# fishmarch/MS-SLAM

Hardware: AMD Instinct MI355X
Metric: Mkeypoints/s extract+describe, KITTI-00-like stereo 1241x376, 2000 feat/frame (higher is better)
Workload: dtype u8

## Files before the change

### ms-slam_amd/csrc/extractor.hip

```cpp
#include <hip/hip_runtime.h>

#include <algorithm>
#include <atomic>
#include <chrono>
#include <condition_variable>
#include <cstdio>
#include <cstdlib>
#include <cstring>
#include <cmath>
#include <functional>
#include <memory>
#include <mutex>
#include <string>
#include <thread>
#include <vector>

#include "frame_io.h"
#include "hip_host.h"
#include "host_admission.h"
#include "orb_device.h"
#include "gauss7_stream_device.h"
#include "matcher_device.h"
#include "stereo_rowtable_device.h"

// ... 4 lines not shown
thread_local std::string g_last_error;

const int8_t kPattern[1024] = {
#include "orb_pattern.inc"
};

class Pool {
    struct Job {
        const std::function<void(int)>* fn;
        int n;
        std::atomic<int> next{0}, done{0};
    };

public:
    explicit Pool(int nthreads) {
        for (int i = 0; i < nthreads - 1; i++) workers_.emplace_back([this] { loop(); });
    }
    ~Pool() {
        {
            std::lock_guard<std::mutex> lk(m_);
            stop_ = true;
        }
        cv_.notify_all();
        for (auto& t : workers_) t.join();
    }
    void parallel_for(int n, const std::function<void(int)>& fn) {
        if (n <= 0) return;
        auto job = std::make_shared<Job>();
        job->fn = &fn;
        job->n = n;
        {
            std::lock_guard<std::mutex> lk(m_);
            cur_ = job;
            gen_++;
        }
        cv_.notify_all();
        work(*job);
        std::unique_lock<std::mutex> lk(m_);
        done_cv_.wait(lk, [&] { return job->done.load() >= n; });
        cur_.reset();
    }

private:
    void work(Job& job) {
        for (;;) {
            const int i = job.next.fetch_add(1);
            if (i >= job.n) break;
            (*job.fn)(i);
            if (job.done.fetch_add(1) + 1 == job.n) {
                std::lock_guard<std::mutex> lk(m_);
                done_cv_.notify_all();
            }
        }
    }
    void loop() {
        unsigned seen = 0;
        for (;;) {
            std::shared_ptr<Job> job;
            {
                std::unique_lock<std::mutex> lk(m_);
                cv_.wait(lk, [&] { return stop_ || gen_ != seen; });
                if (stop_) return;
                seen = gen_;
                job = cur_;
            }
            if (job) work(*job);
        }
    }
    std::vector<std::thread> workers_;
    std::mutex m_;
    std::condition_variable cv_, done_cv_;
    std::shared_ptr<Job> cur_;
    unsigned gen_ = 0;
    bool stop_ = false;
};

}

constexpr int kMaxGroups = 4;
struct StreamGroup {
    hipStream_t s = nullptr;
    bool own_stream = false;
    hipEvent_t ev_pyr = nullptr, ev_blur = nullptr;
    hipEvent_t pe[10] = {};
    bool ready = false;
};

struct msorb_extractor {
    int device = 0;
    StreamGroup grp[kMaxGroups];
    int n_groups = 2;
    bool overlap_blur = true;
    OrbParams P;
    Semantics sem;
    hipStream_t stream = nullptr, copy_stream = nullptr;
    struct Knobs { bool serial_pipeline = false, quadtree_host = false, quadtree_global = false, split_no_peer = false, force_peer_pyramid = false, frame_compact = true; int host_threads = 0, frame_fuse = 2; } knobs;
    int lds_per_block = 64 * 1024;
    bool last_prof = false;
    int pending_batch = 0;
    DevBuf<int> d_st_sad, d_st_rows, d_st_list;
    DevBuf<uint8_t> d_st_block, d_st_img;
    DevBuf<uint8_t> d_out1;
    DevBuf<uint8_t> d_gather_pyr;
    DevBuf<int> d_gather_cnt;
    hipEvent_t ev_split = nullptr;
    bool host_pyramid = false;
    hipStream_t pyr_stream = nullptr;
    bool h_pyr_async = false;
    const uint8_t* pair_l0[2] = {nullptr, nullptr};
    int pair_pyramids = 0;
    unsigned long long buffers_epoch = 0;
    hipEvent_t ev_compact = nullptr;
    bool profiling = false;
    float stage_ms[MSORB_N_STAGES] = {};

    FrameGeom G;
    bool geom_valid = false;
    std::vector<int> level_cell_begin;
    LevelScale scales;

    DevBuf<uint8_t> d_pyr, d_blur;
    DevBuf<ResizeTap> d_taps;
    TowerPlan tower;
    std::vector<size_t> tap_x_off, tap_y_off;
    DevBuf<CellDesc> d_cells;
    DevBuf<FastThreadRec> d_ttab;
    DevBuf<int> d_level_cell_begin, d_cell_count, d_cell_off, d_level_count, d_img_total, d_img_base, d_sel_count;
    DevBuf<Cand16> d_slots, d_compact;
    DevBuf<SelRec> d_sel;
    DevBuf<uint16_t> d_label;
    DevBuf<int> d_sel_pt, d_sel_n, d_mono;
    QtLevels qt{};
    bool device_quadtree = true;
    bool qt_global = false;
    DevBuf<char> d_qt_ws;
    DevBuf<uint32_t> d_label_wide;
    bool small_cells = false;
    bool compact_on_host = false;
    bool compact_fixed_stride = false;
    PinBuf<int> h_level_count, h_img_base, h_sel_count, h_mono;
    PinBuf<Cand16> h_compact;
    PinBuf<SelRec> h_sel;
    PinBuf<uint8_t> h_pyr, h_img_pin, h_out_pin, h_gather;
    bool h_pyr_valid = false;
    bool input_direct = true;
    msorb_input_stats in_stats{};

    PyramidView last_pyr{}, last_blur{};
    int last_n_images = 0;
    int last_groups = 1;
    int sel_stride = 0;

    std::unique_ptr<Pool> pool;
};

namespace {

int frame_copy(void* dst, const void* src, size_t bytes, hipMemcpyKind kind, hipStream_t s) {
    HIPCHK(small_copy(dst, src, bytes, kind, s));
    return MSORB_OK;
}
int capacity_of(const msorb_extractor* h) { return h->P.nfeatures + (3 + 16) * h->P.nlevels; }

bool have_hip_device() {
    int n = 0;
    if (hipGetDeviceCount(&n) == hipSuccess && n > 0) return true;
    (void)hipGetLastError();
// ... 236 lines not shown
    if (h->qt_global && (rc = h->d_qt_ws.ensure((size_t)n_images * g.nlevels * quadtree_global_workspace_stride(h->qt)))) return rc;
    if (h->qt_global && (rc = h->d_label_wide.ensure((size_t)n_images * g.slots_per_image))) return rc;
    if ((rc = h->d_mono.ensure(std::max(n_images, 4)))) return rc;
    return MSORB_OK;
}

PyramidView make_view(const msorb_extractor* h, const uint8_t* base, const LevelView* level0) {
    PyramidView v{};
    const FrameGeom& g = h->G;
    v.nlevels = g.nlevels;
    for (int l = 0; l < g.nlevels; l++) {
        v.lv[l].base = base + g.lv[l].plane_off;
        v.lv[l].img_stride = g.pyramid_bytes;
        v.lv[l].pitch = g.lv[l].pitch;
        v.lv[l].w = g.lv[l].w;
        v.lv[l].h = g.lv[l].h;
    }
    if (level0) v.lv[0] = *level0;
    return v;
}

PyramidView make_blur_view(const msorb_extractor* h, const uint8_t* base) {
    PyramidView v{};
    const FrameGeom& g = h->G;
    v.nlevels = g.nlevels;
    for (int l = 0; l < g.nlevels; l++) {
        v.lv[l].base = base + g.lv[l].blur_off;
        v.lv[l].img_stride = g.blur_bytes;
        v.lv[l].pitch = g.lv[l].pitch;
        v.lv[l].w = g.lv[l].w;
        v.lv[l].h = g.lv[l].h;
    }
    return v;
}

int fetch_candidates(msorb_extractor* h, int n_images) {
    const int nl = h->G.nlevels;
    HIPCHK(hipStreamWaitEvent(h->copy_stream, h->ev_compact, 0));
    HIPCHK(hipMemcpyAsync(h->h_level_count.p, h->d_level_count.p, (size_t)n_images * nl * sizeof(int),
                          hipMemcpyDeviceToHost, h->copy_stream));
    HIPCHK(hipMemcpyAsync(h->h_img_base.p, h->d_img_base.p, (size_t)(n_images + 1) * sizeof(int),
                          hipMemcpyDeviceToHost, h->copy_stream));
    HIPCHK(hipStreamSynchronize(h->copy_stream));
    int rc;
    if (h->compact_fixed_stride) {
        std::vector<int> tot(n_images, 0);
        int total = 0;
        for (int i = 0; i < n_images; i++) {
            for (int l = 0; l < nl; l++) tot[i] += h->h_level_count.p[(size_t)i * nl + l];
            total += tot[i];
        }
        if ((rc = h->h_compact.ensure(std::max<size_t>((size_t)total + total / 4, 1024)))) return rc;
        int at = 0;
        for (int i = 0; i < n_images; i++) {
            if (tot[i] > 0)
                HIPCHK(hipMemcpyAsync(h->h_compact.p + at, h->d_compact.p + (size_t)h->h_img_base.p[i], (size_t)tot[i] * sizeof(Cand16),
                                      hipMemcpyDeviceToHost, h->copy_stream));
            h->h_img_base.p[i] = at;
            at += tot[i];
        }
        h->h_img_base.p[n_images] = at;
        HIPCHK(hipStreamSynchronize(h->copy_stream));
        h->compact_on_host = true;
        return MSORB_OK;
    }
    const int total = h->h_img_base.p[n_images];
    if ((rc = h->h_compact.ensure(std::max<size_t>((size_t)total + total / 4, 1024)))) return rc;
    if (total > 0) {
        HIPCHK(hipMemcpyAsync(h->h_compact.p, h->d_compact.p, (size_t)total * sizeof(Cand16), hipMemcpyDeviceToHost,
                              h->copy_stream));
        HIPCHK(hipStreamSynchronize(h->copy_stream));
    }
    h->compact_on_host = true;
    return MSORB_OK;
}

int ensure_group(msorb_extractor* h, int gi) {
    StreamGroup& G = h->grp[gi];
    if (G.ready) return MSORB_OK;
    if (gi == 0) G.s = h->stream;
    else { HIPCHK(hipStreamCreateWithFlags(&G.s, hipStreamNonBlocking)); G.own_stream = true; }
    HIPCHK(hipEventCreateWithFlags(&G.ev_pyr, hipEventDisableTiming));
    HIPCHK(hipEventCreateWithFlags(&G.ev_blur, hipEventDisableTiming));
    for (auto& e : G.pe) HIPCHK(hipEventCreate(&e));
    G.ready = true;
    return MSORB_OK;
}

bool device_pipeline(const msorb_extractor* h) { return h->device_quadtree && !h->knobs.serial_pipeline; }
bool blur_off_main(const msorb_extractor* h) { return h->overlap_blur && !h->knobs.serial_pipeline; }

struct PipelineCall {
    int lap0 = 0, lap1 = 0;
    int capacity = 0;
    msorb_keypoint* d_kps = nullptr;
    uint8_t* d_desc = nullptr;
    int* h_counts = nullptr;
    int* h_mono = nullptr;
    const StereoRowJob* row_job = nullptr;
    bool defer_sync = false;
    bool skip_count_copies = false;
    int pair_pyramids = 0;
};

int host_pyramid_copies(msorb_extractor* h, int n, hipEvent_t after) {
    const FrameGeom& g = h->G;
    int rc;
    if ((rc = h->h_pyr.ensure((size_t)n * g.pyramid_bytes))) return rc;
    if (!h->pyr_stream) HIPCHK(hipStreamCreateWithFlags(&h->pyr_stream, hipStreamNonBlocking));
    if (after) HIPCHK(hipStreamWaitEvent(h->pyr_stream, after, 0));
    if (g.nlevels > 1)
        for (int i = 0; i < n; i++)
            HIPCHK(hipMemcpyAsync(h->h_pyr.p + (size_t)i * g.pyramid_bytes + g.lv[1].plane_off, h->d_pyr.p + (size_t)i * g.pyramid_bytes + g.lv[1].plane_off,
                                  g.pyramid_bytes - g.lv[1].plane_off, hipMemcpyDeviceToHost, h->pyr_stream));
    h->h_pyr_async = true;
    return MSORB_OK;
}

int finish_groups(msorb_extractor* h, int n_images, int* h_counts, int* h_mono, float host_select_ms = -1.f) {
    const int ng = h->last_groups;
    for (int gi = 0; gi < ng; gi++) HIPCHK(hipStreamSynchronize(h->grp[gi].s));
    HIPCHK(hipGetLastError());
    for (int i = 0; i < n_images; i++) {
        if (h->h_sel_count.p[i] < 0) { set_last_error("keypoint capacity exceeded"); return MSORB_E_CAPACITY; }
        h_counts[i] = h->h_sel_count.p[i];
        if (h_mono) h_mono[i] = h->h_mono.p[i];
    }
    if (h->last_prof) {
        const int fast_from = blur_off_main(h) ? 1 : 8;
        const int map[6][3] = {{MSORB_STAGE_PYRAMID, 0, 1}, {MSORB_STAGE_FAST, fast_from, 2}, {MSORB_STAGE_COMPACT, 2, 3},
                               {MSORB_STAGE_BLUR, 7, 8}, {MSORB_STAGE_SELECT, 3, 5}, {MSORB_STAGE_DESCRIBE, 5, 6}};
        for (auto& m : map) h->stage_ms[m[0]] = 0;
        for (int gi = 0; gi < ng; gi++)
            for (auto& m : map) {
                float ms = 0;
                HIPCHK(hipEventElapsedTime(&ms, h->grp[gi].pe[m[1]], h->grp[gi].pe[m[2]]));
                h->stage_ms[m[0]] += ms;
            }
        if (host_select_ms >= 0) h->stage_ms[MSORB_STAGE_SELECT] = host_select_ms;
    }
    return MSORB_OK;
}

int select_on_host(msorb_extractor* h, int n_images, const PipelineCall& c, hipStream_t s, int* max_sel) {
    const FrameGeom& g = h->G;
    const int nl = g.nlevels, sel_stride = h->sel_stride;
    int rc;
    if ((rc = fetch_candidates(h, n_images))) return rc;
    std::atomic<int> overflow{0};
    std::function<void(int)> task = [&](int img) {
        const Cand16* cand = h->h_compact.p + h->h_img_base.p[img];
        const int* lc = h->h_level_count.p + (size_t)img * nl;
        SelRec* out = h->h_sel.p + (size_t)img * sel_stride;
        std::vector<int> kept;
        int n = 0;
        for (int l = 0; l < nl; l++) {
            const LevelGeom& lg = g.lv[l];
            distribute_quadtree(cand, lc[l], lg.min_x, lg.max_x, lg.min_y, lg.max_y, lg.quota, kept);
            for (int k : kept) {
                if (n >= sel_stride || n >= c.capacity) { overflow.store(1); break; }
                SelRec r;
                r.x = (uint16_t)(cand[k].x + kMinBorder);
                r.y = (uint16_t)(cand[k].y + kMinBorder);
                r.score = cand[k].score;
                r.level = (uint8_t)l;
                r.pad = 0;
                r.dst = 0;
                out[n++] = r;
            }
            cand += lc[l];
        }
        int mono = 0, stereo = n - 1;
        for (int i = 0; i < n; i++) {
            SelRec& r = out[i];
            const float fx = r.level ? (float)r.x * h->P.scale[r.level] : (float)r.x;
            if (fx >= (float)c.lap0 && fx <= (float)c.lap1) r.dst = stereo--;
            else r.dst = mono++;
        }
        h->h_sel_count.p[img] = n;
        h->h_mono.p[img] = mono;
    };
    if (!h->pool) {
        int nthreads = h->knobs.host_threads > 0 ? h->knobs.host_threads : (int)std::thread::hardware_concurrency();
        h->pool.reset(new Pool(std::max(1, std::min(nthreads, 64))));
    }
    h->pool->parallel_for(n_images, task);
    if (overflow.load()) { set_last_error("keypoint capacity exceeded"); return MSORB_E_CAPACITY; }
    *max_sel = 0;
    for (int i = 0; i < n_images; i++) *max_sel = std::max(*max_sel, h->h_sel_count.p[i]);
    HIPCHK(hipMemcpyAsync(h->d_sel.p, h->h_sel.p, (size_t)n_images * sel_stride * sizeof(SelRec), hipMemcpyHostToDevice, s));
    HIPCHK(hipMemcpyAsync(h->d_sel_count.p, h->h_sel_count.p, (size_t)n_images * sizeof(int), hipMemcpyHostToDevice, s));
    return MSORB_OK;
}

int run_pipeline(msorb_extractor* h, const LevelView& level0, int n_images, const PipelineCall& c) {
    const FrameGeom& g = h->G;
    const int nl = g.nlevels;
    const int ncells = (int)g.cells.size();
    const bool prof = h->profiling;
    const bool host_select = !h->device_quadtree;
    const bool overlap_blur = blur_off_main(h);
    const int sel_stride = h->sel_stride;
    int ng = n_images >= 16 && device_pipeline(h) ? std::min(h->n_groups, kMaxGroups) : 1;
    ng = std::max(1, std::min(ng, n_images));
    h->last_pyr = make_view(h, h->d_pyr.p, &level0);
    h->last_blur = make_blur_view(h, h->d_blur.p);
    h->last_n_images = n_images;
    h->pair_pyramids = c.pair_pyramids;
    h->h_pyr_valid = false;
    h->h_pyr_async = false;
    h->compact_on_host = false;
    h->last_groups = ng;
    h->last_prof = prof;
    float host_select_ms = -1.f;
    if (ng > 1) HIPCHK(hipStreamSynchronize(h->stream));
    int first = 0;
    for (int gi = 0; gi < ng; gi++) {
        int rc;
        if ((rc = ensure_group(h, gi))) return rc;
        StreamGroup& G = h->grp[gi];
        const int n = (n_images - first) / (ng - gi);
        hipStream_t s = G.s;
        auto mark = [&](int i, hipStream_t st) { if (prof) (void)hipEventRecord(G.pe[i], st); };
        LevelView l0 = level0;
        l0.base = level0.base + (size_t)first * level0.img_stride;
        uint8_t* pyr_base = h->d_pyr.p + (size_t)first * g.pyramid_bytes;
        const PyramidView pyr = make_view(h, pyr_base, &l0);
        const PyramidView blur = make_blur_view(h, h->d_blur.p + (size_t)first * g.blur_bytes);
        int* img_base = h->d_img_base.p + first + gi;
        const size_t cslot = (size_t)first * g.slots_per_image;
        mark(0, s);
        if (!(n <= 4 && !h->sem.resize_single_stage && launch_pyramid_tower(pyr, h->tower, h->d_taps.p, h->tap_x_off.data(), h->tap_y_off.data(), n, s)))
            launch_pyramid(pyr, h->d_taps.p, h->tap_x_off.data(), h->tap_y_off.data(), n, s, h->sem);
        mark(1, s);
        const bool fuse_ok = ng == 1 && n <= 4 && !prof && overlap_blur && h->sem.default_taps();
        FrameBlurJob blur_job;
        const bool fuse_qt = fuse_ok && !host_select && h->knobs.frame_fuse == 2 && n_images <= 4 && make_frame_blur_job(pyr, blur, n, h->sem, &blur_job);
        const bool fuse_fb = fuse_ok && !fuse_qt && h->knobs.frame_fuse >= 1;
        const bool side_blur = overlap_blur && !fuse_fb && !fuse_qt;
        hipStream_t sb = side_blur ? h->copy_stream : s;
        int host_pyramids = 0;
        if (h->host_pyramid && n_images == 1 && level0.base == h->d_pyr.p + g.lv[0].plane_off) host_pyramids = 1;
        if (h->host_pyramid && n_images == 2 && c.pair_pyramids == 2) host_pyramids = 2;
        if (side_blur || h->host_pyramid) HIPCHK(hipEventRecord(G.ev_pyr, s));
        if (side_blur) HIPCHK(hipStreamWaitEvent(sb, G.ev_pyr, 0));
        if (host_pyramids && (rc = host_pyramid_copies(h, host_pyramids, G.ev_pyr))) return rc;
        bool blur_carried = false;
        auto blur_now = [&]() {
            mark(7, sb);
            (void)launch_gauss7(pyr, blur, n, sb, h->sem);
            mark(8, sb);
            if (side_blur) (void)hipEventRecord(G.ev_blur, sb);
        };
        if (!(fuse_fb && launch_frame_fast_blur(pyr, blur, h->d_cells.p, h->d_ttab.p, ncells, h->P.ini_th, h->P.min_th, g.slots_per_image, h->d_slots.p + cslot,
                                                h->d_cell_count.p + (size_t)first * ncells, n, h->small_cells, s, h->sem))) {
            if (!overlap_blur) blur_now();
            launch_fast_cells(pyr, h->d_cells.p, h->d_ttab.p, ncells, h->P.ini_th, h->P.min_th, g.slots_per_image, h->d_slots.p + cslot,
                              h->d_cell_count.p + (size_t)first * ncells, n, h->small_cells, s);
            mark(2, s);
            if (overlap_blur && !fuse_qt) blur_now();
        }
        launch_cand_compact(h->d_cells.p, ncells, h->d_level_cell_begin.p, nl, g.slots_per_image, h->d_slots.p + cslot,
                            h->d_cell_count.p + (size_t)first * ncells, h->d_cell_off.p + (size_t)first * ncells,
                            h->d_level_count.p + (size_t)first * nl, h->d_img_total.p + first, img_base,
                            h->d_compact.p + cslot, n, s, false, h->knobs.frame_compact && ng == 1);
        h->compact_fixed_stride = true;
        mark(3, s);
        int max_sel = std::min(c.capacity, sel_stride);
        if (host_select) {
            HIPCHK(hipEventRecord(h->ev_compact, s));
            const auto t0 = std::chrono::steady_clock::now();
            if ((rc = select_on_host(h, n, c, s, &max_sel))) return rc;
            host_select_ms = std::chrono::duration<float, std::milli>(std::chrono::steady_clock::now() - t0).count();
        } else {
            if ((rc = launch_quadtree(h->qt, h->d_compact.p + cslot, img_base, h->d_level_count.p + (size_t)first * nl,
                                      h->d_label.p + cslot, h->d_sel_pt.p + (size_t)first * sel_stride, h->d_sel_n.p + (size_t)first * nl,
                                      sel_stride, h->scales, c.lap0, c.lap1, c.capacity, h->d_sel.p + (size_t)first * sel_stride,
                                      h->d_sel_count.p + first, h->d_mono.p + first, n, s, ng == 1 ? c.row_job : nullptr,
                                      fuse_qt ? &blur_job : nullptr, &blur_carried,
                                      h->qt_global ? h->d_qt_ws.p + (size_t)first * nl * quadtree_global_workspace_stride(h->qt) : nullptr,
                                      h->qt_global ? h->d_label_wide.p + cslot : nullptr)))
                return rc;
            if (fuse_qt && !blur_carried) blur_now();
        }
        mark(5, s);
        if (side_blur) HIPCHK(hipStreamWaitEvent(s, G.ev_blur, 0));
        launch_describe(pyr, blur, h->d_sel.p + (size_t)first * sel_stride, h->d_sel_count.p + first, sel_stride, h->scales,
                        c.d_kps + (size_t)first * c.capacity, c.d_desc + (size_t)first * c.capacity * 32, c.capacity, max_sel, n, s, h->sem);
        mark(6, s);
        if (!c.skip_count_copies && !host_select) {
            if (n_images <= 4 && first == 0) {
                int crc;
                if ((crc = frame_copy(h->h_sel_count.p, h->d_sel_count.p, (size_t)n * sizeof(int), hipMemcpyDeviceToHost, s)) ||
                    (crc = frame_copy(h->h_mono.p, h->d_mono.p, (size_t)n * sizeof(int), hipMemcpyDeviceToHost, s)))
                    return crc;
            } else {
                HIPCHK(hipMemcpyAsync(h->h_sel_count.p + first, h->d_sel_count.p + first, (size_t)n * sizeof(int), hipMemcpyDeviceToHost, s));
                HIPCHK(hipMemcpyAsync(h->h_mono.p + first, h->d_mono.p + first, (size_t)n * sizeof(int), hipMemcpyDeviceToHost, s));
            }
        }
        first += n;
    }
    if (c.defer_sync) return MSORB_OK;
    return finish_groups(h, n_images, c.h_counts, c.h_mono, host_select_ms);
}

StereoBatchArgs stereo_frame_args(const msorb_extractor* h, const FrameBlock& fb, uint8_t* blk, const PyramidView& right, const int* counts_right,
                                  int rows, float mb, float mbf) {
    StereoBatchArgs b{};
    b.A.kpL = reinterpret_cast<msorb_keypoint*>(blk + fb.o_kps(0)); b.A.kpR = reinterpret_cast<msorb_keypoint*>(blk + fb.o_kps(1));
    b.A.descL = blk + fb.o_descs(0); b.A.descR = blk + fb.o_descs(1);
    b.countsL = h->d_sel_count.p; b.countsR = counts_right;
    b.A.rows0 = rows;
    for (int l = 0; l < h->G.nlevels; l++) {
        const LevelView &vl = h->last_pyr.lv[l], &vr = right.lv[l];
        b.A.pyrL[l] = vl.base; b.A.pyrR[l] = vr.base;
        b.A.pitchL[l] = vl.pitch; b.A.pitchR[l] = vr.pitch;
        b.A.rows[l] = vl.h; b.A.cols[l] = vl.w;
        b.A.scale[l] = h->scales.scale[l]; b.A.inv_scale[l] = h->P.inv_scale[l];
        b.img_strideL[l] = vl.img_stride; b.img_strideR[l] = vr.img_stride;
    }
    b.A.mb = mb; b.A.mbf = mbf;
    b.A.u_right = reinterpret_cast<float*>(blk + fb.o_ur); b.A.depth = reinterpret_cast<float*>(blk + fb.o_dp);
    b.A.sad = h->d_st_sad.p; b.A.n_oob = reinterpret_cast<int*>(blk + fb.o_oob);
    b.capacity = (int)fb.cap;
    b.counts_out = reinterpret_cast<int*>(blk + fb.o_cnt);
    return b;
}

}

namespace msorb {
void set_last_error(const std::string& s) { g_last_error = s; }
int extractor_last_view(msorb_extractor* h, PyramidView* pyr, LevelScale* sc, float* inv_scale, int* device,
                        hipStream_t* stream, int* n_images) {
    if (!h || !h->geom_valid || h->last_n_images < 1) {
        set_last_error("extractor has no pyramid yet (call msorb_extract first)");
        return MSORB_E_INVALID;
    }
    *pyr = h->last_pyr;
    if (sc) *sc = h->scales;
// ... 67 lines not shown
    return MSORB_OK;
}

int msorb_device_count(void) {
    int n = 0;
    if (hipGetDeviceCount(&n) != hipSuccess) return 0;
    return n;
}

int msorb_device_memory(int device, size_t* free_bytes, size_t* total_bytes) {
    if (!free_bytes || !total_bytes) return MSORB_E_INVALID;
    HIPCHK(hipSetDevice(device));
    HIPCHK(hipMemGetInfo(free_bytes, total_bytes));
    return MSORB_OK;
}

int msorb_extractor_create(int nfeatures, float scale_factor, int nlevels, int ini_th, int min_th, int device,
                           msorb_extractor** out) {
    if (!out) return MSORB_E_INVALID;
    *out = nullptr;
    if (nfeatures <= 0 || nlevels < 1 || nlevels > MSORB_MAX_LEVELS || !(scale_factor > 1.0f) || ini_th < 0 ||
        min_th < 0 || ini_th > 255 || min_th > ini_th) {
        set_last_error("invalid extractor parameters");
        return MSORB_E_INVALID;
    }
    if (int rc = require_device(device)) return rc;
    HIPCHK(hipSetDevice(device));
    msorb_extractor* h = new msorb_extractor();
    h->device = device;
    h->P.init(nfeatures, scale_factor, nlevels, ini_th, min_th);
    for (int l = 0; l < nlevels; l++) {
        h->scales.scale[l] = h->P.scale[l];
        h->scales.patch[l] = (float)(int)(kPatchSize * h->P.scale[l]);
    }
    int prio_least = 0, prio_greatest = 0;
    (void)hipDeviceGetStreamPriorityRange(&prio_least, &prio_greatest);
    const int prio_blur = prio_least;
    if (hipStreamCreateWithFlags(&h->stream, hipStreamNonBlocking) != hipSuccess ||
        hipStreamCreateWithPriority(&h->copy_stream, hipStreamNonBlocking, prio_blur) != hipSuccess ||
        hipEventCreateWithFlags(&h->ev_compact, hipEventDisableTiming) != hipSuccess) {
        set_last_error("stream/event creation failed");
        delete h;
        return MSORB_E_HIP;
    }
    upload_patch_tables(kPattern, h->P.umax, h->stream);
    {
        const char* e;
        h->knobs.serial_pipeline = getenv("MSORB_SERIAL_PIPELINE") != nullptr;
        h->knobs.quadtree_host = (e = getenv("MSORB_QUADTREE")) && std::string(e) == "host";
        h->knobs.quadtree_global = (e = getenv("MSORB_QUADTREE")) && std::string(e) == "global";
        h->knobs.split_no_peer = getenv("MSORB_SPLIT_NO_PEER") != nullptr;
        h->knobs.force_peer_pyramid = getenv("MSORB_FORCE_PEER_PYRAMID") != nullptr;
        h->knobs.host_threads = (e = getenv("MSORB_HOST_THREADS")) ? atoi(e) : 0;
        h->knobs.frame_fuse = (e = getenv("MSORB_FRAME_FUSE")) ? std::max(0, std::min(2, atoi(e))) : 2;
        h->knobs.frame_compact = !((e = getenv("MSORB_FRAME_COMPACT")) && e[0] == '0');
        h->input_direct = !((e = getenv("MSORB_INPUT_DIRECT")) && e[0] == '0');
    }
    if (hipDeviceGetAttribute(&h->lds_per_block, hipDeviceAttributeMaxSharedMemoryPerBlock, device) != hipSuccess || h->lds_per_block <= 0)
        h->lds_per_block = 64 * 1024;
    *out = h;
    return MSORB_OK;
}

void msorb_extractor_destroy(msorb_extractor* h) {
    if (!h) return;
    (void)hipSetDevice(h->device);
    if (h->stream) (void)hipStreamSynchronize(h->stream);
    h->pool.reset();
    h->d_pyr.release(); h->d_blur.release(); h->d_taps.release(); h->d_cells.release(); h->d_ttab.release();
    h->d_level_cell_begin.release(); h->d_cell_count.release(); h->d_cell_off.release(); h->d_level_count.release();
    h->d_img_total.release(); h->d_img_base.release(); h->d_sel_count.release(); h->d_slots.release();
    h->d_compact.release(); h->d_sel.release();
    h->d_st_sad.release(); h->d_st_rows.release(); h->d_st_list.release(); h->d_st_block.release(); h->d_st_img.release(); h->d_out1.release();
    h->d_gather_pyr.release(); h->d_gather_cnt.release();
    if (h->ev_split) (void)hipEventDestroy(h->ev_split);
    if (h->pyr_stream) { (void)hipStreamSynchronize(h->pyr_stream); (void)hipStreamDestroy(h->pyr_stream); }
    h->h_level_count.release(); h->h_img_base.release(); h->h_sel_count.release(); h->h_compact.release();
    h->h_sel.release(); h->h_pyr.release(); h->h_img_pin.release(); h->h_out_pin.release(); h->h_gather.release();
    for (auto& G : h->grp) {
        if (!G.ready) continue;
        (void)hipStreamSynchronize(G.s);
        for (auto& e : G.pe) if (e) (void)hipEventDestroy(e);
        (void)hipEventDestroy(G.ev_pyr); (void)hipEventDestroy(G.ev_blur);
        if (G.own_stream) (void)hipStreamDestroy(G.s);
    }
    if (h->ev_compact) (void)hipEventDestroy(h->ev_compact);
    if (h->stream) (void)hipStreamDestroy(h->stream);
    if (h->copy_stream) (void)hipStreamDestroy(h->copy_stream);
    delete h;
}

int msorb_extractor_tables(const msorb_extractor* h, float* scale, float* inv_scale, float* sigma2, float* inv_sigma2,
                           int* per_level) {
    if (!h) return MSORB_E_INVALID;
    for (int l = 0; l < h->P.nlevels; l++) {
        if (scale) scale[l] = h->P.scale[l];
        if (inv_scale) inv_scale[l] = h->P.inv_scale[l];
        if (sigma2) sigma2[l] = h->P.sigma2[l];
        if (inv_sigma2) inv_sigma2[l] = h->P.inv_sigma2[l];
        if (per_level) per_level[l] = h->P.per_level[l];
    }
    return MSORB_OK;
}

int msorb_extractor_capacity(const msorb_extractor* h) { return h ? capacity_of(h) : MSORB_E_INVALID; }

int msorb_extractor_set_profiling(msorb_extractor* h, int enable) {
    if (!h) return MSORB_E_INVALID;
    h->profiling = enable != 0;
    return MSORB_OK;
}
int msorb_extractor_set_overlap(msorb_extractor* h, int sub_batches, int blur_on_second_stream) {
    if (!h || sub_batches < 1 || sub_batches > kMaxGroups) return MSORB_E_INVALID;
    h->n_groups = sub_batches;
    h->overlap_blur = blur_on_second_stream != 0;
    return MSORB_OK;
}
int msorb_extractor_set_semantics(msorb_extractor* h, const msorb_semantics* sem) {
    if (!h) return MSORB_E_INVALID;
    if (h->pending_batch) { set_last_error("a submitted batch of this handle has not been waited for"); return MSORB_E_INVALID; }
    Semantics s;
    if (sem) {
        int sum = 0;
        for (int i = 0; i < 7; i++) {
            if (sem->gauss_taps[i] < 0 || sem->gauss_taps[i] > 255) { set_last_error("gauss tap outside 0..255"); return MSORB_E_INVALID; }
            s.gauss_taps[i] = sem->gauss_taps[i];
            sum += sem->gauss_taps[i];
        }
        if (sum < 1 || sum > 257) { set_last_error("gauss taps: the 16-bit horizontal sums need sum(taps) <= 257"); return MSORB_E_INVALID; }
        s.resize_single_stage = sem->resize_rounding != 0;
        s.atan2_fma = sem->atan2_fma != 0;
        if (sem->brief_tap < 0 || sem->brief_tap > 2) { set_last_error("brief_tap must be 0 (first product fused), 1 (second product fused) or 2 (no contraction)"); return MSORB_E_INVALID; }
        s.brief_tap = sem->brief_tap;
    }
    h->sem = s;
    return MSORB_OK;
}

int msorb_extractor_set_host_pyramid(msorb_extractor* h, int enable) {
    if (!h) return MSORB_E_INVALID;
    h->host_pyramid = enable != 0;
    return MSORB_OK;
}
int msorb_extractor_stage_ms(const msorb_extractor* h, float* ms) {
    if (!h || !ms) return MSORB_E_INVALID;
    for (int i = 0; i < MSORB_N_STAGES; i++) ms[i] = h->stage_ms[i];
    return MSORB_OK;
}

static int extract_batch_common(msorb_extractor* h, const uint8_t* d_images, int n_images, int rows, int cols, size_t row_stride,
                                size_t image_stride, int lap0, int lap1, msorb_keypoint* d_kps, uint8_t* d_desc, int capacity,
                                int* h_counts, int* h_mono, bool submit_only) {
    if (!h || !d_kps || !d_desc || (!submit_only && !h_counts) || n_images < 0) { set_last_error("null argument"); return MSORB_E_INVALID; }
    if (h->pending_batch) { set_last_error("a submitted batch of this handle has not been waited for"); return MSORB_E_INVALID; }
    if (!d_images || rows <= 0 || cols <= 0) return MSORB_E_EMPTY;
    if (n_images == 0) return MSORB_OK;
    if ((int)row_stride < cols || (n_images > 1 && image_stride < row_stride * (size_t)rows)) {
        set_last_error("bad strides");
        return MSORB_E_INVALID;
    }
    if (submit_only && !device_pipeline(h)) {
        set_last_error("msorb_extract_batch_submit needs the device pipeline");
        return MSORB_E_INVALID;
    }
    HIPCHK(hipSetDevice(h->device));
    int rc;
// ... 585 lines not shown
```

### ms-slam_amd/csrc/orb_device.h

```cpp
#pragma once
#include <hip/hip_runtime.h>
#include <stdint.h>

#include <string>
#include <vector>

#include "../../include/msorb.h"
#include "orb_host.h"

namespace msorb {
void set_last_error(const std::string& s);

struct LevelView {
    const uint8_t* base;
    size_t img_stride;
    int pitch, w, h;
};
__host__ __device__ inline uint32_t blur_tile_off(uint32_t x, uint32_t y, uint32_t pitch) {
    return (y >> 2) * (pitch * 4u) + (x >> 2) * 16u + (y & 3u) * 4u + (x & 3u);
}
struct PyramidView {
    LevelView lv[kMaxLevels];
    int nlevels;
};
struct LevelScale {
    float scale[kMaxLevels];
    float patch[kMaxLevels];
};
struct SelRec {
    uint16_t x, y, score;
    uint8_t level, pad;
    int32_t dst;
};

struct QtLevels {
    int W[kMaxLevels], H[kMaxLevels], quota[kMaxLevels], n_ini[kMaxLevels];
    int sel_off[kMaxLevels];
    int nlevels;
};

struct StereoRowJob;
struct FrameBlurJob;
int launch_quadtree(const QtLevels& lv, const Cand16* compact, const int* img_base, const int* level_count,
                     uint16_t* label, int* sel_pt, int* sel_n, int sel_stride, const LevelScale& scales, int lap0,
                     int lap1, int capacity, SelRec* sel, int* sel_count, int* mono, int n_images, hipStream_t s,
                     const StereoRowJob* row_job = nullptr, const FrameBlurJob* blur_job = nullptr, bool* blur_carried = nullptr,
                     char* global_ws = nullptr, uint32_t* global_label = nullptr);
size_t quadtree_global_workspace_stride(const QtLevels& lv);
void launch_quadtree_select_global(const QtLevels& lv, const Cand16* compact, const int* img_base, const int* level_count, uint32_t* label, int* sel_pt,
                                   int* sel_n, int sel_stride, int n_images, char* ws, hipStream_t s);
size_t quadtree_lds_bytes(const QtLevels& lv);
int launch_debug_sort(const uint32_t* h_keys, int n, int frame_form, uint32_t* h_nodes, uint32_t* h_keys_out, float* sort_us);
int launch_debug_cos_sin(const float* h_angles_deg, int n, float* h_cos, float* h_sin);
void upload_patch_tables(const int8_t* pattern, const int* umax, hipStream_t stream);
hipError_t download_patch_tables(int8_t* pattern , int8_t* umax , hipStream_t stream);
void launch_blit(void* dst, const void* src, size_t bytes, hipStream_t s);
hipError_t small_copy(void* dst, const void* src, size_t bytes, hipMemcpyKind kind, hipStream_t s);
void launch_stage_level0(const LevelView& src, uint8_t* dst, int dst_pitch, size_t dst_image_stride, int n_images, hipStream_t s);
struct Level0Src { const uint8_t* base; size_t stride; };
void launch_upload_level0(const Level0Src* src, int n_images, uint8_t* dst, size_t dst_image_stride, int dst_pitch, int rows, int cols, hipStream_t s);
struct Semantics {
    int gauss_taps[7] = {18, 34, 48, 56, 48, 34, 18};
    int resize_single_stage = 0;
    int atan2_fma = 0;
    int brief_tap = 0;
    bool default_taps() const {
        static const int d[7] = {18, 34, 48, 56, 48, 34, 18};
        for (int i = 0; i < 7; i++) if (gauss_taps[i] != d[i]) return false;
        return true;
    }
};
constexpr int kTowerTiles = 16;
struct TowerAxis {
    int16_t need0[kTowerTiles], need1[kTowerTiles];
};
__host__ __device__ inline int tower_own_x(int k, int n, int w) { return k >= n ? (w + 3) & ~3 : (int)((long long)k * w / n) & ~3; }
__host__ __device__ inline int tower_own_y(int k, int n, int h) { return k >= n ? h : (int)((long long)k * h / n); }
struct TowerPlan {
    TowerAxis x[kMaxLevels], y[kMaxLevels];
    int ntx = 0, nty = 0;
    int lds_even = 0, lds_odd = 0;
    int lds_taps = 0;
};
bool build_tower_plan(TowerPlan& plan, int nlevels, const int* w, const int* h, const int* pitch, const std::vector<std::vector<ResizeTap>>& taps_x,
                      const std::vector<std::vector<ResizeTap>>& taps_y, size_t lds_limit);
bool launch_pyramid_tower(const PyramidView& pyr, const TowerPlan& plan, const ResizeTap* taps, const size_t* tap_x_off, const size_t* tap_y_off,
                          int n_images, hipStream_t s);
void launch_pyramid(const PyramidView& pyr, const ResizeTap* taps, const size_t* tap_x_off, const size_t* tap_y_off, int n_images,
                    hipStream_t s, const Semantics& sem = Semantics());
void launch_pyr_resize(const LevelView& src, const LevelView& dst, uint8_t* dst_base, const ResizeTap* tx,
                       const ResizeTap* ty, int n_images, hipStream_t s, int single_stage = 0);
void launch_fast_cells(const PyramidView& pyr, const CellDesc* cells, const FastThreadRec* ttab, int n_cells, int ini_th, int min_th,
                       int slots_per_image, Cand16* slots, int* cell_count, int n_images, bool small_cells, hipStream_t s);
void launch_cand_compact(const CellDesc* cells, int n_cells, const int* level_cell_begin, int nlevels,
                         int slots_per_image, const Cand16* slots, const int* cell_count, int* cell_off,
                         int* level_count, int* img_total, int* img_base, Cand16* compact, int n_images,
                         hipStream_t s, bool packed = true, bool frame_form = false);
int launch_gauss7(const PyramidView& src, const PyramidView& dst, int n_images, hipStream_t s, const Semantics& sem = Semantics());
bool launch_frame_fast_blur(const PyramidView& pyr, const PyramidView& blur, const CellDesc* cells, const FastThreadRec* ttab, int n_cells, int ini_th, int min_th,
                            int slots_per_image, Cand16* slots, int* cell_count, int n_images, bool small_cells, hipStream_t s,
                            const Semantics& sem = Semantics());
void launch_describe(const PyramidView& pyr, const PyramidView& blur, const SelRec* sel, const int* sel_count,
                     int sel_stride, const LevelScale& scales, msorb_keypoint* kps, uint8_t* desc, int out_stride,
                     int max_sel, int n_images, hipStream_t s, const Semantics& sem = Semantics());

}
```

### ms-slam_amd/csrc/orb_kernels.hip

```cpp
#include <hip/hip_runtime.h>

#include <algorithm>
#include <string>
#include <stdint.h>
#include <stdlib.h>

#include "lds_limit.h"
#include "orb_device.h"
#include "gauss7_stream_device.h"
#include "sincosf_restated.h"

namespace msorb {

__global__ __launch_bounds__(256) void pyr_resize_kernel(LevelView src, LevelView dst, uint8_t* __restrict__ dst_base,
                                                         const ResizeTap* __restrict__ tx,
                                                         const ResizeTap* __restrict__ ty, int single_stage) {
    const int img = blockIdx.z;
    const int dy = blockIdx.y * 4 + (threadIdx.x >> 6);
    const int dx0 = (blockIdx.x * 64 + (threadIdx.x & 63)) * 4;
    if (dy >= dst.h || dx0 >= dst.w) return;
    const ResizeTap vy = ty[dy];
    const uint8_t* s0 = src.base + (size_t)img * src.img_stride + (size_t)vy.i0 * src.pitch;
    const uint8_t* s1 = src.base + (size_t)img * src.img_stride + (size_t)vy.i1 * src.pitch;
    const int b0 = vy.c0, b1 = vy.c1;
// ... 1453 lines not shown
                const int sh = (i1 != i0) ? 8 : 0;
                const int h0 = (int)(pa & 255u) * c0 + (int)((pa >> sh) & 255u) * c1;
                const int h1 = (int)(pb & 255u) * c0 + (int)((pb >> sh) & 255u) * c1;
                const int v = (((b0 * (h0 >> 4)) >> 16) + ((b1 * (h1 >> 4)) >> 16) + 2) >> 2;
                if (dx0 + k < dw) packed |= (uint32_t)(v & 255) << (8 * k);
            }
            *reinterpret_cast<uint32_t*>(dbuf + r * dp + 4 * c) = packed;
            if (dy >= oy0 && dy < oy1 && dx0 >= ox0 && dx0 < ox1) *reinterpret_cast<uint32_t*>(dplane + (size_t)dy * dpitch + dx0) = packed;
        }
        __syncthreads();
    }
}

bool build_tower_plan(TowerPlan& plan, int nlevels, const int* w, const int* h, const int* pitch, const std::vector<std::vector<ResizeTap>>& taps_x,
                      const std::vector<std::vector<ResizeTap>>& taps_y, size_t lds_limit) {
    plan = TowerPlan{};
    if (nlevels < 2) return false;
    const int ntx = kTowerTiles, nty = w[0] >= 2 * h[0] ? kTowerTiles / 2 : kTowerTiles;
    for (int l = 0; l < nlevels; l++)
        if (pitch[l] < ((w[l] + 3) & ~3)) return false;
    size_t lds[2] = {0, 0};
    for (int tyi = 0; tyi < kTowerTiles; tyi++)
        for (int l = nlevels - 1; l >= 0; l--) {
            int a = l ? tower_own_y(tyi, nty, h[l]) : 32767, b = l ? tower_own_y(tyi + 1, nty, h[l]) : -1;
            if (l + 1 < nlevels && plan.y[l + 1].need1[tyi] > plan.y[l + 1].need0[tyi]) {
                const auto& t = taps_y[l + 1];
                a = std::min<int>(a, t[plan.y[l + 1].need0[tyi]].i0);
                b = std::max<int>(b, t[std::min<int>(plan.y[l + 1].need1[tyi], h[l + 1]) - 1].i1 + 1);
            }
            if (b <= a) { a = 0; b = 0; }
            plan.y[l].need0[tyi] = (int16_t)a; plan.y[l].need1[tyi] = (int16_t)b;
        }
    for (int txi = 0; txi < kTowerTiles; txi++)
        for (int l = nlevels - 1; l >= 0; l--) {
            int a = l ? tower_own_x(txi, ntx, w[l]) : 32767, b = l ? tower_own_x(txi + 1, ntx, w[l]) : -1;
            if (l + 1 < nlevels && plan.x[l + 1].need1[txi] > plan.x[l + 1].need0[txi]) {
                const auto& t = taps_x[l + 1];
                a = std::min<int>(a, t[std::min<int>(plan.x[l + 1].need0[txi], w[l + 1] - 1)].i0);
                b = std::max<int>(b, (t[std::min<int>(plan.x[l + 1].need1[txi], w[l + 1]) - 1].i1 + 1));
            }
            if (b <= a) { a = 0; b = 0; }
            a &= ~3; b = (b + 3) & ~3;
            plan.x[l].need0[txi] = (int16_t)a; plan.x[l].need1[txi] = (int16_t)b;
        }
    for (int l = 0; l < nlevels; l++)
        for (int tyi = 0; tyi < nty; tyi++)
            for (int txi = 0; txi < ntx; txi++) {
                const size_t bytes = (size_t)(plan.x[l].need1[txi] - plan.x[l].need0[txi] + 8) * (plan.y[l].need1[tyi] - plan.y[l].need0[tyi]) + 16;
                lds[l & 1] = std::max(lds[l & 1], (bytes + 15) & ~size_t(15));
            }
    size_t n_taps = 0;
    for (int tyi = 0; tyi < nty; tyi++)
        for (int txi = 0; txi < ntx; txi++) {
            size_t t = 0;
            for (int l = 1; l < nlevels; l++) t += (size_t)(plan.x[l].need1[txi] - plan.x[l].need0[txi]) + ((plan.y[l].need1[tyi] - plan.y[l].need0[tyi] + 1) & ~1);
            n_taps = std::max(n_taps, t);
        }
    if (n_taps > 2048 || lds[0] + lds[1] + (n_taps + 8) * sizeof(ResizeTap) > lds_limit) return false;
    plan.ntx = ntx; plan.nty = nty;
    plan.lds_even = (int)lds[0]; plan.lds_odd = (int)lds[1]; plan.lds_taps = (int)((n_taps + 8) * sizeof(ResizeTap));
    return true;
}
bool launch_pyramid_tower(const PyramidView& pyr, const TowerPlan& plan, const ResizeTap* taps, const size_t* tap_x_off, const size_t* tap_y_off,
                          int n_images, hipStream_t s) {
    static const bool off = getenv("MSORB_PYR_TOWER") && atoi(getenv("MSORB_PYR_TOWER")) == 0;
    const LevelView& v0 = pyr.lv[0];
    if (off || plan.ntx <= 0 || (reinterpret_cast<uintptr_t>(v0.base) & 3) || (v0.pitch & 3) || (v0.img_stride & 3) || v0.pitch < ((v0.w + 3) & ~3) ||
        (reinterpret_cast<uintptr_t>(taps) & 31))
        return false;
    const size_t lds = (size_t)plan.lds_even + plan.lds_odd + plan.lds_taps;
    if ((long long)lds > dynamic_lds_room(reinterpret_cast<const void*>(pyr_tower_kernel))) return false;
    TowerTaps t{};
    for (int l = 1; l < pyr.nlevels; l++) { t.x[l] = taps + tap_x_off[l]; t.y[l] = taps + tap_y_off[l]; }
    hipLaunchKernelGGL(pyr_tower_kernel, dim3(plan.ntx, plan.nty, n_images), dim3(kTowerThreads), lds, s, pyr, plan, t);
    return true;
}
void launch_pyramid(const PyramidView& pyr, const ResizeTap* taps, const size_t* tap_x_off, const size_t* tap_y_off, int n_images,
                    hipStream_t s, const Semantics& sem) {
    for (int l = 1; l < pyr.nlevels; l++)
        launch_pyr_resize(pyr.lv[l - 1], pyr.lv[l], const_cast<uint8_t*>(pyr.lv[l].base), taps + tap_x_off[l], taps + tap_y_off[l], n_images, s,
                          sem.resize_single_stage);
}
void launch_fast_cells(const PyramidView& pyr, const CellDesc* cells, const FastThreadRec* ttab, int n_cells, int ini_th, int min_th,
                       int slots_per_image, Cand16* slots, int* cell_count, int n_images, bool small_cells, hipStream_t s) {
    bool aligned = true;
    for (int l = 0; l < pyr.nlevels; l++) {
        const LevelView& v = pyr.lv[l];
        aligned = aligned && (reinterpret_cast<uintptr_t>(v.base) & 3) == 0 && (v.pitch & 3) == 0 && (v.img_stride & 3) == 0;
    }
    const dim3 grid(n_cells, n_images);
    const uint32_t gx_magic = exact_div_magic((unsigned)n_cells, (unsigned long long)n_cells * (unsigned)n_images);
#define MSORB_FAST_LAUNCH(AL, GEO)                                                                                        \
    hipLaunchKernelGGL((fast_cells_kernel<AL, GEO>), grid, dim3(GEO::kThreads), 0, s, pyr, cells, ttab, ini_th, min_th, slots_per_image, slots, \
                       cell_count, n_cells, gx_magic)
    if (small_cells) { if (aligned) MSORB_FAST_LAUNCH(true, GeoSmall); else MSORB_FAST_LAUNCH(false, GeoSmall); }
    else { if (aligned) MSORB_FAST_LAUNCH(true, GeoLarge); else MSORB_FAST_LAUNCH(false, GeoLarge); }
#undef MSORB_FAST_LAUNCH
}
void launch_cand_compact(const CellDesc* cells, int n_cells, const int* level_cell_begin, int nlevels,
                         int slots_per_image, const Cand16* slots, const int* cell_count, int* cell_off,
                         int* level_count, int* img_total, int* img_base, Cand16* compact, int n_images,
                         hipStream_t s, bool packed, bool frame_form) {
    if (!packed && frame_form && n_images <= 4 && n_cells <= kFrameCompactCells) {
        hipLaunchKernelGGL(cand_compact_frame_kernel, dim3((n_cells + kGatherCells - 1) / kGatherCells, n_images), dim3(kGatherThreads), 0, s, cells, n_cells,
                           level_cell_begin, nlevels, slots_per_image, slots, cell_count, cell_off, level_count, img_total, img_base, compact);
        return;
    }
    hipLaunchKernelGGL(cand_scan_cells_kernel, dim3(n_images), dim3(256), 0, s, cell_count, n_cells, level_cell_begin,
                       nlevels, cell_off, level_count, img_total, img_base, packed ? 0 : slots_per_image);
    if (packed) hipLaunchKernelGGL(cand_scan_images_kernel, dim3(1), dim3(256), 0, s, img_total, n_images, img_base);
    hipLaunchKernelGGL(cand_gather_kernel, dim3((n_cells + kGatherCells - 1) / kGatherCells, n_images), dim3(kGatherThreads), 0, s, cells, n_cells, slots_per_image,
                       slots, cell_count, cell_off, img_base, compact);
}
static bool levels_aligned(const PyramidView& v) {
    bool aligned = true;
    for (int l = 0; l < v.nlevels; l++) {
        const LevelView& lv = v.lv[l];
        aligned = aligned && (reinterpret_cast<uintptr_t>(lv.base) & 3) == 0 && (lv.pitch & 3) == 0 && (lv.img_stride & 3) == 0;
    }
    return aligned;
}
static BlurPlan make_blur_plan(const PyramidView& src, int n_images, bool stream, int* total_out, int* max_h_out) {
    BlurPlan plan{};
    plan.nlevels = src.nlevels;
    const int rows = kGaussRows;
    int total = 0, max_h = 0;
    for (int l = 0; l < src.nlevels; l++) {
        const LevelView& v = src.lv[l];
        plan.block_begin[l] = total;
        const int main_groups = stream ? (v.w + 3) / 4 : (v.w >= 16 ? (v.w - 16) / 4 + 1 : 0);
        plan.bx_count[l] = stream ? max(1, (main_groups - 1 + kGaussLanesOut - 1) / kGaussLanesOut) : (v.w + 255) / 256;
        const int strips = (v.h + rows - 1) / rows;
        total += plan.bx_count[l] * ((strips + 3) / 4);
        max_h = max(max_h, v.h);
    }
    plan.block_begin[src.nlevels] = total;
    for (int l = 0; l < src.nlevels; l++)
        plan.bx_magic[l] = exact_div_magic((unsigned)plan.bx_count[l], (unsigned long long)(plan.block_begin[l + 1] - plan.block_begin[l]));
    for (int l = src.nlevels; l < kMaxLevels; l++) plan.bx_magic[l] = 0;
    plan.image_magic = exact_div_magic((unsigned)total, (unsigned long long)total * (unsigned)n_images + 8);
    *total_out = total;
    *max_h_out = max_h;
    return plan;
}
int launch_gauss7(const PyramidView& src, const PyramidView& dst, int n_images, hipStream_t s, const Semantics& sem) {
    const bool aligned = levels_aligned(src);
    const bool stream = aligned && sem.default_taps();
    GaussTaps T;
    for (int i = 0; i < 7; i++) T.k[i] = (uint32_t)sem.gauss_taps[i];
    int total = 0, max_h = 0;
    const BlurPlan plan = make_blur_plan(src, n_images, stream, &total, &max_h);
    if (stream) {
        const int all = total * n_images, per_xcd = (all + 7) / 8;
        hipLaunchKernelGGL(gauss7_stream_kernel<kGaussRows>, dim3(per_xcd * 8), dim3(256), 0, s, src, dst, plan, per_xcd, all);
    }
    else if (aligned) hipLaunchKernelGGL(gauss7_kernel<true>, dim3(total, n_images), dim3(256), 0, s, src, dst, plan, T);
    else hipLaunchKernelGGL(gauss7_kernel<false>, dim3(total, n_images), dim3(256), 0, s, src, dst, plan, T);
    if (!stream)
        hipLaunchKernelGGL(gauss7_edge_kernel, dim3((max_h + kEdgeRows - 1) / kEdgeRows, src.nlevels, n_images), dim3(64), 0, s, src, dst, T);
    return 0;
}
bool make_frame_blur_job(const PyramidView& src, const PyramidView& dst, int n_images, const Semantics& sem, FrameBlurJob* job) {
    if (!levels_aligned(src) || !sem.default_taps()) return false;
    int total = 0, max_h = 0;
    job->src = src; job->dst = dst;
    job->plan = make_blur_plan(src, n_images, true, &total, &max_h);
    job->blocks = total * n_images;
    return true;
}
bool launch_frame_fast_blur(const PyramidView& pyr, const PyramidView& blur, const CellDesc* cells, const FastThreadRec* ttab, int n_cells, int ini_th, int min_th,
                            int slots_per_image, Cand16* slots, int* cell_count, int n_images, bool small_cells, hipStream_t s,
                            const Semantics& sem) {
    if (!levels_aligned(pyr) || !sem.default_taps()) return false;
    int total = 0, max_h = 0;
// ... 29 lines not shown
```

Before: 501.2.

## Overlap FAST detection on early pyramid levels with pyramid build on side stream

For batches larger than four images, FAST corner detection for level 0 (and level 1 once it is resized) now launches on a side stream while the main stream builds the remaining pyramid levels. The remaining levels run FAST on the main stream, which then waits on the side stream's event. launch_fast_cells gains a cell range so it can run on a subset of levels, and the profiling map records a per-group FAST start. The aim is to hide FAST latency behind pyramid resizing. The cost is extra events, cross-stream waits, and a per-level resize path that replaces the tower kernel in that case.

```diff
diff --git a/ms-slam_amd/csrc/extractor.hip b/ms-slam_amd/csrc/extractor.hip
--- a/ms-slam_amd/csrc/extractor.hip
+++ b/ms-slam_amd/csrc/extractor.hip
@@ -110,7 +110,9 @@
     hipStream_t s = nullptr;
     bool own_stream = false;
     hipEvent_t ev_pyr = nullptr, ev_blur = nullptr;
+    hipEvent_t ev_begin = nullptr, ev_l1 = nullptr, ev_fast0 = nullptr;
     hipEvent_t pe[10] = {};
+    int fast_from = 1;
     bool ready = false;
 };
 
@@ -513,6 +515,9 @@
     else { HIPCHK(hipStreamCreateWithFlags(&G.s, hipStreamNonBlocking)); G.own_stream = true; }
     HIPCHK(hipEventCreateWithFlags(&G.ev_pyr, hipEventDisableTiming));
     HIPCHK(hipEventCreateWithFlags(&G.ev_blur, hipEventDisableTiming));
+    HIPCHK(hipEventCreateWithFlags(&G.ev_begin, hipEventDisableTiming));
+    HIPCHK(hipEventCreateWithFlags(&G.ev_fast0, hipEventDisableTiming));
+    HIPCHK(hipEventCreateWithFlags(&G.ev_l1, hipEventDisableTiming));
     for (auto& e : G.pe) HIPCHK(hipEventCreate(&e));
     G.ready = true;
     return MSORB_OK;
@@ -558,16 +563,17 @@
         if (h_mono) h_mono[i] = h->h_mono.p[i];
     }
     if (h->last_prof) {
-        const int fast_from = blur_off_main(h) ? 1 : 8;
-        const int map[6][3] = {{MSORB_STAGE_PYRAMID, 0, 1}, {MSORB_STAGE_FAST, fast_from, 2}, {MSORB_STAGE_COMPACT, 2, 3},
-                               {MSORB_STAGE_BLUR, 7, 8}, {MSORB_STAGE_SELECT, 3, 5}, {MSORB_STAGE_DESCRIBE, 5, 6}};
+        int map[6][3] = {{MSORB_STAGE_PYRAMID, 0, 1}, {MSORB_STAGE_FAST, 1, 2}, {MSORB_STAGE_COMPACT, 2, 3},
+                         {MSORB_STAGE_BLUR, 7, 8}, {MSORB_STAGE_SELECT, 3, 5}, {MSORB_STAGE_DESCRIBE, 5, 6}};
         for (auto& m : map) h->stage_ms[m[0]] = 0;
-        for (int gi = 0; gi < ng; gi++)
+        for (int gi = 0; gi < ng; gi++) {
+            map[1][1] = h->grp[gi].fast_from;
             for (auto& m : map) {
                 float ms = 0;
                 HIPCHK(hipEventElapsedTime(&ms, h->grp[gi].pe[m[1]], h->grp[gi].pe[m[2]]));
                 h->stage_ms[m[0]] += ms;
             }
+        }
         if (host_select_ms >= 0) h->stage_ms[MSORB_STAGE_SELECT] = host_select_ms;
     }
     return MSORB_OK;
@@ -660,10 +666,36 @@
         const PyramidView blur = make_blur_view(h, h->d_blur.p + (size_t)first * g.blur_bytes);
         int* img_base = h->d_img_base.p + first + gi;
         const size_t cslot = (size_t)first * g.slots_per_image;
+        auto fast_levels = [&](int l_first, int l_end, hipStream_t st) {
+            launch_fast_cells(pyr, h->d_cells.p, h->d_ttab.p, ncells, h->P.ini_th, h->P.min_th, g.slots_per_image, h->d_slots.p + cslot,
+                              h->d_cell_count.p + (size_t)first * ncells, n, h->small_cells, st, h->level_cell_begin[l_first],
+                              h->level_cell_begin[l_end] - h->level_cell_begin[l_first]);
+        };
+        const bool head = overlap_blur && n > 4;
+        const int side_levels = !head ? 0 : nl >= 3 ? 2 : 1;
+        hipStream_t side = h->copy_stream;
+        G.fast_from = head ? 4 : overlap_blur ? 1 : 8;
+        if (head) {
+            HIPCHK(hipEventRecord(G.ev_begin, s));
+            HIPCHK(hipStreamWaitEvent(side, G.ev_begin, 0));
+            mark(4, side);
+            fast_levels(0, 1, side);
+        }
         mark(0, s);
-        if (!(n <= 4 && !h->sem.resize_single_stage && launch_pyramid_tower(pyr, h->tower, h->d_taps.p, h->tap_x_off.data(), h->tap_y_off.data(), n, s)))
+        if (side_levels == 2) {
+            for (int l = 1; l < nl; l++) {
+                launch_pyr_resize(pyr.lv[l - 1], pyr.lv[l], const_cast<uint8_t*>(pyr.lv[l].base), h->d_taps.p + h->tap_x_off[l], h->d_taps.p + h->tap_y_off[l], n, s,
+                                  h->sem.resize_single_stage);
+                if (l == 1) {
+                    HIPCHK(hipEventRecord(G.ev_l1, s));
+                    HIPCHK(hipStreamWaitEvent(side, G.ev_l1, 0));
+                    fast_levels(1, 2, side);
+                }
+            }
+        } else if (!(n <= 4 && !h->sem.resize_single_stage && launch_pyramid_tower(pyr, h->tower, h->d_taps.p, h->tap_x_off.data(), h->tap_y_off.data(), n, s)))
             launch_pyramid(pyr, h->d_taps.p, h->tap_x_off.data(), h->tap_y_off.data(), n, s, h->sem);
         mark(1, s);
+        if (head) HIPCHK(hipEventRecord(G.ev_fast0, side));
         const bool fuse_ok = ng == 1 && n <= 4 && !prof && overlap_blur && h->sem.default_taps();
         FrameBlurJob blur_job;
         const bool fuse_qt = fuse_ok && !host_select && h->knobs.frame_fuse == 2 && n_images <= 4 && make_frame_blur_job(pyr, blur, n, h->sem, &blur_job);
@@ -686,8 +718,8 @@
         if (!(fuse_fb && launch_frame_fast_blur(pyr, blur, h->d_cells.p, h->d_ttab.p, ncells, h->P.ini_th, h->P.min_th, g.slots_per_image, h->d_slots.p + cslot,
                                                 h->d_cell_count.p + (size_t)first * ncells, n, h->small_cells, s, h->sem))) {
             if (!overlap_blur) blur_now();
-            launch_fast_cells(pyr, h->d_cells.p, h->d_ttab.p, ncells, h->P.ini_th, h->P.min_th, g.slots_per_image, h->d_slots.p + cslot,
-                              h->d_cell_count.p + (size_t)first * ncells, n, h->small_cells, s);
+            fast_levels(side_levels, nl, s);
+            if (head) HIPCHK(hipStreamWaitEvent(s, G.ev_fast0, 0));
             mark(2, s);
             if (overlap_blur && !fuse_qt) blur_now();
         }
@@ -921,6 +953,7 @@
         (void)hipStreamSynchronize(G.s);
         for (auto& e : G.pe) if (e) (void)hipEventDestroy(e);
         (void)hipEventDestroy(G.ev_pyr); (void)hipEventDestroy(G.ev_blur);
+        (void)hipEventDestroy(G.ev_begin); (void)hipEventDestroy(G.ev_fast0); (void)hipEventDestroy(G.ev_l1);
         if (G.own_stream) (void)hipStreamDestroy(G.s);
     }
     if (h->ev_compact) (void)hipEventDestroy(h->ev_compact);
diff --git a/ms-slam_amd/csrc/orb_device.h b/ms-slam_amd/csrc/orb_device.h
--- a/ms-slam_amd/csrc/orb_device.h
+++ b/ms-slam_amd/csrc/orb_device.h
@@ -91,7 +91,8 @@
 void launch_pyr_resize(const LevelView& src, const LevelView& dst, uint8_t* dst_base, const ResizeTap* tx,
                        const ResizeTap* ty, int n_images, hipStream_t s, int single_stage = 0);
 void launch_fast_cells(const PyramidView& pyr, const CellDesc* cells, const FastThreadRec* ttab, int n_cells, int ini_th, int min_th,
-                       int slots_per_image, Cand16* slots, int* cell_count, int n_images, bool small_cells, hipStream_t s);
+                       int slots_per_image, Cand16* slots, int* cell_count, int n_images, bool small_cells, hipStream_t s,
+                       int cell_first = 0, int cell_n = -1);
 void launch_cand_compact(const CellDesc* cells, int n_cells, const int* level_cell_begin, int nlevels,
                          int slots_per_image, const Cand16* slots, const int* cell_count, int* cell_off,
                          int* level_count, int* img_total, int* img_base, Cand16* compact, int n_images,
diff --git a/ms-slam_amd/csrc/orb_kernels.hip b/ms-slam_amd/csrc/orb_kernels.hip
--- a/ms-slam_amd/csrc/orb_kernels.hip
+++ b/ms-slam_amd/csrc/orb_kernels.hip
@@ -1559,14 +1559,19 @@
                           sem.resize_single_stage);
 }
 void launch_fast_cells(const PyramidView& pyr, const CellDesc* cells, const FastThreadRec* ttab, int n_cells, int ini_th, int min_th,
-                       int slots_per_image, Cand16* slots, int* cell_count, int n_images, bool small_cells, hipStream_t s) {
+                       int slots_per_image, Cand16* slots, int* cell_count, int n_images, bool small_cells, hipStream_t s,
+                       int cell_first, int cell_n) {
+    if (cell_n < 0) cell_n = n_cells - cell_first;
+    if (cell_first < 0 || cell_n <= 0 || cell_first + cell_n > n_cells || n_images <= 0) return;
     bool aligned = true;
     for (int l = 0; l < pyr.nlevels; l++) {
         const LevelView& v = pyr.lv[l];
         aligned = aligned && (reinterpret_cast<uintptr_t>(v.base) & 3) == 0 && (v.pitch & 3) == 0 && (v.img_stride & 3) == 0;
     }
-    const dim3 grid(n_cells, n_images);
-    const uint32_t gx_magic = exact_div_magic((unsigned)n_cells, (unsigned long long)n_cells * (unsigned)n_images);
+    cells += cell_first;
+    cell_count += cell_first;
+    const dim3 grid(cell_n, n_images);
+    const uint32_t gx_magic = exact_div_magic((unsigned)cell_n, (unsigned long long)cell_n * (unsigned)n_images);
 #define MSORB_FAST_LAUNCH(AL, GEO)                                                                                        \
     hipLaunchKernelGGL((fast_cells_kernel<AL, GEO>), grid, dim3(GEO::kThreads), 0, s, pyr, cells, ttab, ini_th, min_th, slots_per_image, slots, \
                        cell_count, n_cells, gx_magic)
```

Measured after the change: 507.8, median of 4. 1.3% higher.
